# mit-acl/faster

Measured on AMD Instinct MI355X. Metric: trajectory solves/sec (whole+safe pairs) at N=10, deg=3, higher is better.
Workload: dtype f64; 1 GPU; C4: 32768 whole+safe paired solves per GPU per step (N=10 segments, deg=3, <=6 polytopes whole / <=3 safe), synthetic corridors (faster_amd/corridor.py seed 3), hand-off keeps R >= 0.05 m inside its safe corridor; pairs_per_gpu=32768, pipeline=fused, pipelines_in_flight=14, parallelism=single GPU

## Files before the change

### faster_amd/csrc/fh_solve.hip.hpp

```cpp
#pragma once
#include <hip/hip_runtime.h>
#include <stdint.h>

#include "../../include/fasterhip.h"
#include "fh_basis.hip.hpp"
#include "fh_share.hip.hpp"
#include "fh_sample.hip.hpp"

namespace fh {

#ifndef FH_LOOK_EVERY
#define FH_LOOK_EVERY 8
#endif
#ifndef FH_LOOK_EVERY_BUSY
#define FH_LOOK_EVERY_BUSY 16
#endif

#define FH_SYNC() __builtin_amdgcn_fence(__ATOMIC_SEQ_CST, "wavefront")
__device__ __forceinline__ unsigned long long pinned_clock() {
  unsigned long long t;
  asm volatile("s_memtime %0\n\ts_waitcnt lgkmcnt(0)" : "=s"(t) : : "memory");
  return t;
}
#ifdef FH_PROFILE
// ... 212 lines not shown
  const float a0 = (float)x0a, v0 = (float)x0v;
  const double c3 = (double)jerk / 6.0, c2 = (double)a0 / 2.0, c1 = (double)v0, c0 = -dx;
  double ic3 = __builtin_amdgcn_rcp(c3);
  ic3 = fma(fma(-c3, ic3, 1.0), ic3, ic3);
  const double B = c2 * ic3, C = c1 * ic3, D = c0 * ic3, B3 = B * (1.0 / 3.0);
  const double p = C - B * B3;
  const double q = 2.0 * B3 * B3 * B3 - B3 * C + D;
  const double q2 = 0.5 * q, p3 = p * (1.0 / 3.0);
  const double p27 = p3 * p3 * p3;
  const double disc = q2 * q2 + p27;
  const double scale = q2 * q2 + fabs(p27);
  const float acc = (float)(copysign(1.0, dx) * pr.a_max);
  const double qc2 = 0.5 * (double)acc;
  const double qdisc = c1 * c1 - 4.0 * qc2 * c0;
  const bool triple = !(disc > 0) && p == 0;
  const bool ill = !(fabs(disc) >= 1e-6 * scale) || (scale > 0.0 && scale < 1e-40) || !(scale < 1e280) || !(qdisc >= 0.0) || (triple && B != 0.0) ||
                   !(fabs(dx) >= 1e-30);
  if (wave_any(ill && lane < 12)) return dt_initial_exact_lanes(pr, x0, opaque(lane));
  double rj = 0.0;
  if (disc > 0) {
    const double sq = __builtin_amdgcn_sqrt(disc);
    const double u = cbrt_start(sq - q2), v = cbrt_start(-q2 - sq);
    rj = u + v - B3;
  } else if (triple) {
    rj = 0.0;
  } else {
    const double m = 2.0 * __builtin_amdgcn_sqrt(-p3);
    const float arg = fminf(1.0f, fmaxf(-1.0f, (float)(3.0 * q * __builtin_amdgcn_rcp(p * m))));
    const float rev = acos_start(arg) * (1.0f / (3.0f * 6.28318531f)) - (float)j * (1.0f / 3.0f);
    rj = m * (double)__builtin_amdgcn_cosf(rev) - B3;
  }
  if (!triple) {
#pragma unroll
    for (int it = 0; it < 3; it++) {
      const double f = ((c3 * rj + c2) * rj + c1) * rj + c0;
      const double df = (3 * c3 * rj + 2 * c2) * rj + c1;
      double r = __builtin_amdgcn_rcp(df);
      r = fma(fma(-df, r, 1.0), r, r);
      const double tn = rj - f * r;
      rj = (df == 0 || !isfinite(df) || !isfinite(tn)) ? rj : tn;
    }
  }
  if (((disc > 0 || triple) && j != 0) || j == 3) rj = 0.0;
  double ra = 0.0;
  {
    const double sr = sqrt(qdisc);
    const double qq = -0.5 * (c1 + (c1 >= 0 ? sr : -sr));
    if (qq != 0) ra = j == 0 ? qq / qc2 : (j == 1 ? c0 / qq : 0.0);
  }
  double mj = rj > 0 ? rj : INFINITY, ma = ra > 0 ? ra : INFINITY;
  mj = vmin_f64(mj, dpp_f64<0xB1, 0xf>(INFINITY, mj));
  ma = vmin_f64(ma, dpp_f64<0xB1, 0xf>(INFINITY, ma));
  mj = vmin_f64(mj, dpp_f64<0x4E, 0xf>(INFINITY, mj));
  ma = vmin_f64(ma, dpp_f64<0x4E, 0xf>(INFINITY, ma));
  const float tj = (float)(mj < INFINITY ? mj : 0.0), ta = (float)(ma < INFINITY ? ma : 0.0);
  const float ml = fmaxf(tv, fmaxf(ta, tj));
  const int mli = __float_as_int(ml);
  const float mx = fmaxf(fmaxf(0.f, __int_as_float(__builtin_amdgcn_readlane(mli, 0))),
                         fmaxf(__int_as_float(__builtin_amdgcn_readlane(mli, 4)), __int_as_float(__builtin_amdgcn_readlane(mli, 8))));
  double dt0 = (double)(mx / (float)pr.n_seg);
  if (dt0 > 10000) dt0 = 0;
  return dt0;
#endif
}

typedef const __attribute__((address_space(3))) double lds_cdouble;
__device__ __attribute__((noinline)) void write_safe_problem(const fh_problem* whole, const fh_face* wfaces, fh_problem* ps, fh_face* sfaces, lds_cdouble* x0P,
                                                             int x0_stride, int start, int cnt, double shrink, double r_margin, int lane) {
  lds_cdouble* x0V = x0P + x0_stride;
  lds_cdouble* x0A = x0V + x0_stride;
  const double x0[9] = {x0P[0], x0P[1], x0P[2], x0V[0], x0V[1], x0V[2], x0A[0], x0A[1], x0A[2]};
  const int fb = __builtin_amdgcn_readfirstlane(whole->face_begin);
  glue_write_safe<true>(wfaces, fb, whole->face_off, start, cnt, x0, shrink, r_margin, *ps, sfaces, lane, nullptr);
}

template <int NSEG>
struct Solver {
  static constexpr int NX = 3 * NSEG;
  static constexpr int NXP = (NX + 7) & ~7;
  static constexpr int KMAX = NSEG - 2;
  static constexpr int NV = 3 * KMAX;
  static constexpr int NVP = (NV + 7) & ~7;
  static constexpr int S = NVP + 1;
  static constexpr int NT = NSEG + 1;
  static constexpr int ZS = NSEG | 1;
  static_assert(NSEG >= 3, "reduced space needs N - 2 > 0 columns");
  static constexpr bool HALF = 3 * NSEG <= 32;
  static __device__ __forceinline__ double lo_sum(double v) {
    if constexpr (HALF) return half_sum(v);
    else return wave_sum(v);
  }
  static __device__ __forceinline__ double lo_min(double v) {
    if constexpr (HALF) return half_min(v);
    else return wave_min(v);
  }
  static __device__ __forceinline__ void lo_sum2(double a, double b, double& sa, double& sb) {
    if constexpr (HALF) half_sum2(a, b, sa, sb);
    else { sa = wave_sum(a); sb = wave_sum(b); }
  }
  static constexpr int RPSZ = NVP * (NVP + 1) / 2;
  static __device__ __forceinline__ int rp(int r_, int c_) { return (c_ * (c_ + 1)) / 2 + r_; }

  double *Q, *R;
  double *x, *z, *g, *d, *r, *u, *rinv;
  double *tcache, *tbnd;
  static constexpr int TC = NSEG <= 6 ? 2 : 0;
  double* xs;
  double* Zm;
  double *Pc, *Vc, *Ac;
  double* viol;
  double* xfl;
  float* tolf;
  fh_face* faces;
  int *act, *assign, *bestassign, *fullassign, *stk_seg, *stk_next, *stk_cnt, *stk_q, *stk_mask, *stk_keep, *face_off;
  int* tb;
  enum { TB_B = 0, TB_PHASE = 1, TB_F = 2, TB_TRIALS = 4, TB_BASE = 5, TB_H = 7, TB_REC = 9, TB_DEPTH0 = 10, TB_KEY = 11, TB_QE = 13,
         TB_T0 = 14, TB_WORK = 16, TB_ZN = 17, TB_NEXT = 18, TB_NEXT_EI = 20, TB_NEXT_WT = 22, TB_DONE_N = 24, TB_DONE_IT = 25, TB_SAFE = 26, TB_POOL2 = 27, TB_FRESH = 29, TB_WORDS = 30 };
  signed char* stk_order;

  static __host__ __device__ constexpr size_t lds_bytes(int max_faces) {
    return sizeof(double) * (NVP * S + RPSZ + 3 * NVP + NVP / 2 + 2 * NVP + NXP + NSEG * ZS + 3 * NT * 3 + 12 + TC * (2 * NVP + NVP / 2 + FH_MAX_POLY)) +
           sizeof(int) * (9 * NSEG + FH_MAX_POLY + 1 + TB_WORDS) + ((NSEG * FH_MAX_POLY + 15) & ~15) +
           (sizeof(fh_face) + sizeof(float)) * max_faces + 16;
  }

  double p0r, v0r, a0r;
  double xpr;
  double xj;
  double wbj, wbv, wba, wcp;
  double* bestx_g;
  double cp_r[3];
  int scan_f0, scan_F;
  int lane, N, n, q, P;
  int nx;
  int K, zc0;
  int qe;
  bool eq_ok;
  double c0;
  double box_ub;
  double gx2;
  int maxF;
  int scan_trip;
  unsigned poly_ok;
#ifdef FH_PROFILE
  unsigned long long prof[24];
  unsigned int cnt[24];
  unsigned long long take_cycles; unsigned int take_calls;
  unsigned long long glue_parts[4];
  unsigned long long pre_cycles, glue_cycles, drain_cycles;
  unsigned long long prof2[12];
  unsigned long long pre_parts[3];
#endif
  unsigned allowed_first, allowed_last;
  double h, tol, dep2;
  double vmax, amax, jmax;
  int force_final;


  __device__ void carve(unsigned char* base, int max_faces) {
    double* p = reinterpret_cast<double*>(base);
    Q = p; p += NVP * S;
    R = p; p += RPSZ;
    x = p; p += NVP;  u = p; p += NVP;
    act = reinterpret_cast<int*>(p); p += NVP / 2;
    rinv = p; p += NVP;
    g = p; p += NVP;  d = p; p += NVP;  r = d;
    xs = p; p += NXP;
    z = xs;
    static_assert(NXP >= NVP, "z aliases xs");
    Zm = p; p += NSEG * ZS;
    Pc = p; p += NT * 3;  Vc = p; p += NT * 3;  Ac = p; p += NT * 3;
    viol = g;
    static_assert(NSEG * FH_MAX_POLY <= 2 * NVP + NXP && 9 <= NVP, "scratch must fit in g,d,xs");
    xfl = p; p += 12;
    tcache = p; p += TC * SNAP_TAIL;
    tbnd = p; p += TC * FH_MAX_POLY;
    int* ip = reinterpret_cast<int*>(p);
    assign = ip; ip += NSEG;  bestassign = ip; ip += NSEG;  fullassign = ip; ip += NSEG;
    stk_seg = ip; ip += NSEG;  stk_next = ip; ip += NSEG;  stk_cnt = ip; ip += NSEG;  stk_q = ip; ip += NSEG;  stk_mask = ip; ip += NSEG;  stk_keep = ip; ip += NSEG;
    face_off = ip; ip += FH_MAX_POLY + 1;
    tb = ip; ip += TB_WORDS;
    stk_order = reinterpret_cast<signed char*>(ip);
    const size_t off = (size_t)(reinterpret_cast<unsigned char*>(ip) - base) + NSEG * FH_MAX_POLY;
    faces = reinterpret_cast<fh_face*>(base + ((off + 15) & ~(size_t)15));
    tolf = reinterpret_cast<float*>(faces + max_faces);
  }

  static constexpr int SNAP_TAIL = 2 * NVP + NVP / 2;
  static constexpr int SNAP_QOFF = (SNAP_TAIL + 127) & ~127;
  static constexpr int SNAP_BOUNDS = SNAP_TAIL, SNAP_TAIL_COPY = SNAP_TAIL + FH_MAX_POLY;
  static_assert(SNAP_TAIL + FH_MAX_POLY <= ((SNAP_TAIL + 127) & ~127), "the child bounds live in the padding behind the tail");
  static constexpr int SNAP_ROFF = SNAP_QOFF + ((NVP * S + 127) & ~127) + 128;
  static constexpr int SNAP_PADDED = SNAP_ROFF + ((RPSZ + 127) & ~127) + 128;
  __device__ __forceinline__ void copy_out(double* __restrict__ dst, const double* src, int count) const {
    const int n2 = (count + 1) >> 1;
    const double2* s2 = reinterpret_cast<const double2*>(src);
    double2* d2 = reinterpret_cast<double2*>(dst);
    for (int i = lane; i < n2; i += 64) d2[i] = s2[i];
  }
  __device__ __forceinline__ void copy_in(double* dst, const double* __restrict__ src, int count) const {
    const int n2 = (count + 1) >> 1;
    double2* d2 = reinterpret_cast<double2*>(dst);
    const double2* s2 = reinterpret_cast<const double2*>(src);
    for (int i0 = 0; i0 < n2; i0 += 256) {
      double2 t[4];
#pragma unroll
      for (int j = 0; j < 4; j++) {
        const int i = i0 + j * 64 + lane;
        t[j] = s2[i < n2 ? i : 0];
      }
#pragma unroll
      for (int j = 0; j < 4; j++) {
        const int i = i0 + j * 64 + lane;
        if (i < n2) d2[i] = t[j];
      }
    }
  }
  __device__ void snapshot_save(double* __restrict__ ws_level, int level) {
    const int lane = opaque(this->lane);
    FH_SYNC();
    if (level < TC) {
      double* tc = tcache + level * SNAP_TAIL;
      for (int i = lane; i < SNAP_TAIL; i += 64) tc[i] = x[i];
    } else {
      copy_out(ws_level, x, SNAP_TAIL);
    }
    copy_out(ws_level + SNAP_QOFF, Q, q * S);
    copy_out(ws_level + SNAP_ROFF, R, (q * (q + 1)) / 2);
    if (lane == 0) stk_keep[level] = q;
  }
  __device__ void snapshot_restore(const double* __restrict__ ws_level, int q_saved, int level) {
    const int lane = opaque(this->lane);
    const int keep0 = uniform_i32(stk_keep[level]);
    const bool intact = keep0 >= q_saved;
    const bool cached = level < TC;
    int keep = keep0 < 0 ? 0 : (keep0 > q_saved ? q_saved : keep0);
    keep &= ~1;
    if (!cached || !intact) __builtin_amdgcn_fence(__ATOMIC_SEQ_CST, "workgroup");
    if (lane < NVP)
      for (int c = q_saved; c < q; c++) Q[c * S + lane] = 0.0;
    FH_SYNC();
    constexpr int TAIL2 = SNAP_TAIL / 2, TAIL_TRIPS = (TAIL2 + 63) / 64;
    static_assert(SNAP_TAIL % 2 == 0, "the tail is copied 16 B at a time");
    if (!intact) {
      const int r0 = ((keep * (keep + 1)) / 2) & ~1;
      const int nr = (q_saved * (q_saved + 1)) / 2 - r0, nr2 = (nr + 1) >> 1;
      const double2* st2 = reinterpret_cast<const double2*>(ws_level);
      const double2* sr2 = reinterpret_cast<const double2*>(ws_level + SNAP_ROFF + r0);
      double2 tail[TAIL_TRIPS];
      if (!cached) {
#pragma unroll
        for (int j = 0; j < TAIL_TRIPS; j++) tail[j] = st2[(j * 64 + lane) < TAIL2 ? j * 64 + lane : 0];
      }
      double2 rr[2];
#pragma unroll
      for (int j = 0; j < 2; j++) rr[j] = sr2[(j * 64 + lane) < nr2 ? j * 64 + lane : 0];
      copy_in(Q + keep * S, ws_level + SNAP_QOFF + keep * S, (q_saved - keep) * S);
      if (!cached) {
#pragma unroll
        for (int j = 0; j < TAIL_TRIPS; j++)
          if (j * 64 + lane < TAIL2) reinterpret_cast<double2*>(x)[j * 64 + lane] = tail[j];
      }
#pragma unroll
      for (int j = 0; j < 2; j++)
        if (j * 64 + lane < nr2) reinterpret_cast<double2*>(R + r0)[j * 64 + lane] = rr[j];
      if (nr2 > 128) copy_in(R + r0 + 256, ws_level + SNAP_ROFF + r0 + 256, nr - 256);
    } else if (!cached) {
      copy_in(x, ws_level, SNAP_TAIL);
    }
    if (cached) {
      const double* tc = tcache + level * SNAP_TAIL;
      for (int i = lane; i < SNAP_TAIL; i += 64) x[i] = tc[i];
    }
    q = q_saved;
    if (lane == 0) stk_keep[level] = q_saved;
    FH_SYNC();
    if (lane < q_saved) rinv[lane] = 1.0 / R[rp(lane, lane)];
    FH_SYNC();
  }

  __device__ void init_problem() {
    const int lane = opaque(this->lane);
    for (int i = lane; i < NVP * S; i += 64) Q[i] = 0.0;
    for (int i = lane; i < RPSZ; i += 64) R[i] = 0.0;
    if (lane < NVP) { x[lane] = 0; g[lane] = 0; d[lane] = 0; u[lane] = 0; rinv[lane] = 0; act[lane] = 0; }
    if (lane < NXP) xs[lane] = 0;
    q = 0;
    FH_SYNC();
  }

  __device__ __forceinline__ void moments(double& dp, double& dv, double& da) const {
#pragma clang fp contract(off)
    const int lane = opaque(this->lane);
    double s0 = 0, s1 = 0, s2 = 0;
    if constexpr (HALF) {
      static_assert(!HALF || NSEG % 2 == 0, "the two halves take NSEG / 2 segments each");
      constexpr int H = NSEG / 2;
      const int row = lane & 31, hh = lane >> 5;
      const int t1 = row / 3, i = row - 3 * t1;
      const double* xh = xs + 3 * H * hh + (row < 3 * NSEG ? i : 0);
      double xr[H];
#pragma unroll
      for (int s = 0; s < H; s++) xr[s] = xh[3 * s];
      in_flight(xr);
      const int lim = opaque(t1 + 1 - H * hh);
      const double dm0 = (double)(lim - 1);
// ... 594 lines not shown
    q--;
    FH_SYNC();
  }

  __device__ void reset_qp() {
    const int lane = opaque(this->lane);
    if (lane < NVP) {
      for (int c = 0; c < q; c++) Q[c * S + lane] = 0.0;
      x[lane] = 0;
    }
    q = 0;
    FH_SYNC();
  }

  __device__ int qp_run(double ub, bool tie, int max_iters, int& iters, double& cost) {
    int it = 0;
    if (lane == 0) tb[TB_FRESH] = 0;
    bind_assignment();
    const int q0 = q;
    const int st = qp_loop(ub, tie, max_iters, it, cost);
    iters += it;
    const int qa = (q0 + q) >> 1;
    flops += (unsigned long long)(unsigned)(it + 1) * (unsigned)(2 * nx * K + 3 * (N + 1) * (5 * N + 9) + 48 * N + 18 * N + 7 * rows4 + 4 * nx + 2 * n * N) +
             (unsigned long long)(unsigned)it * (unsigned)(4 * n * qa + qa * qa + 4 * n + 5 * qa);
    return st;
  }
  __device__ int qp_loop(double ub, bool tie, int max_iters, int& it, double& cost) {
    for (;;) {
      { FH_T0(); compute_states(); FH_T1(2); }
      int id;
      double vp;
      {
        FH_T0();
        {
          const double xl = (lane < n) ? x[lane] : 0.0;
          double x2, l1x;
          lo_sum2(xl * xl, fabs(xj), x2, l1x);
          cost = c0 + x2;
          if (!(cost <= box_ub) || cost > l1x * (jmax + tol) * (1.0 + 1e-9)) {
            const int al = lane < NVP ? act[lane] : 0;
            conflict = wave_or((lane < q && (al >> 24) == K_POLY) ? (1u << ((al >> 16) & 31)) : 0u);
            return 1;
          }
          if (cost > ub || (tie && cost == ub)) return 2;
        }
        bool cbad;
        scan(id, vp, cbad);
        FH_T1(3);
        if (cbad) return 1;
        if (id < 0) return 0;
      }
      double gg;
      { FH_T0(); gg = build_g(id); FH_T1(4); }
      double up = 0;
      for (;;) {
        if (++it > max_iters) return 3;
        double dc, zi, zz, rc;
        { FH_T0(); zz = project(gg, dc, zi); FH_T1(5); }
        FH_T0();
        rc = backsolve(dc);
        const bool dependent = zz <= dep2 * gx2;
        double ratio = INFINITY;
        if (lane < q && rc > 0) ratio = u[lane] / rc;
        const double t1 = wave_any(ratio < INFINITY) ? lo_min(ratio) : INFINITY;
        const int kb = (t1 < INFINITY) ? first_lane(ratio == t1) : -1;
        if (kb < 0 && dependent) {
          const int al = lane < NVP ? act[lane] : 0;
          bool in = lane < q && rc != 0.0;
          if (vp * (1.0 - 1e-9) > tol) {
            double cn = 0.0;
            const int cl = lane < q ? lane : 0;
            for (int r_ = 0; r_ < q; r_++) {
              const double v = R[rp(min(r_, cl), cl)];
              cn += (r_ <= cl) ? v * v : 0.0;
            }
            const double xl = (lane < n) ? x[lane] : 0.0;
            const double xn = sqrt(wave_sum(xl * xl));
            const double thr = 1e-9 * vp / ((double)q * (xn + sqrt((double)nx) * jmax));
            in = in && fabs(rc) * sqrt(cn) > thr;
          }
          conflict = wave_or((in && (al >> 24) == K_POLY) ? (1u << ((al >> 16) & 31)) : 0u) |
                     ((id >> 24) == K_POLY ? (1u << ((id >> 16) & 31)) : 0u);
          return 1;
        }
        const double t2 = dependent ? INFINITY : vp / zz;
        const double t = fmin(t1, t2);
        if (lane < q) u[lane] -= t * rc;
        up += t;
        if (!dependent) {
          if (lane < n) x[lane] -= t * zi;
          vp -= t * zz;
        }
        FH_T1(6);
        if (t2 <= t1) {
          FH_T0();
          add_row(id, zi, zz, dc, up);
#ifdef FH_QMAX_STAT
          qmax = max(qmax, q);
#endif
          FH_T1(7);
          break;
        }
        FH_SYNC();
        { FH_T0(); drop_row(kb); FH_T1(8); }
      }
    }
  }

  __device__ __forceinline__ unsigned allowed_mask(int t) const {
    unsigned m = P ? (((1u << P) - 1u) & poly_ok) : 0u;
    if (t == 0) m &= allowed_first;
    if (t == N - 1) m &= allowed_last;
    return m;
  }

  template <class PR>
  __device__ void screen_constant_rows(const PR& pr) {
    const int lane = opaque(this->lane);
    allowed_first = allowed_last = 0xffffffffu;
    if (P == 0) return;
    double c0[9], cN[9];
    {
      const double h3 = h / 3.0, h23 = 2.0 * h / 3.0, h26 = h * h / 6.0;
#pragma unroll
      for (int i = 0; i < 3; i++) {
        const double p0 = Pc[i], v0 = Vc[i], a0 = Ac[i];
        const double pf = xfl[i], vf = xfl[3 + i], af = xfl[6 + i];
        c0[i] = p0; c0[3 + i] = p0 + v0 * h3; c0[6 + i] = p0 + v0 * h23 + a0 * h26;
        cN[i] = pf; cN[3 + i] = pf - vf * h3; cN[6 + i] = pf - vf * h23 + af * h26;
      }
    }
    const int nf = face_off[P];
    unsigned bad = 0u;
    for (int fb = 0; fb < nf; fb += 64) {
      const int f = fb + lane;
      const bool valid = f < nf;
      const fh_face fc = faces[valid ? f : 0];
      double w0 = -INFINITY, wN = -INFINITY;
#pragma unroll
      for (int k = 0; k < 3; k++) {
        w0 = vmax_f64(w0, fma(fc.a[0], c0[3 * k], fma(fc.a[1], c0[3 * k + 1], fma(fc.a[2], c0[3 * k + 2], fc.b))));
        wN = vmax_f64(wN, fma(fc.a[0], cN[3 * k], fma(fc.a[1], cN[3 * k + 1], fma(fc.a[2], cN[3 * k + 2], fc.b))));
      }
      int pf = 0;
      for (int j = 1; j < P; j++) pf += (f >= face_off[j]) ? 1 : 0;
      if (valid) bad |= ((w0 > 0.0) ? (1u << pf) : 0u) | ((wN > 0.0) ? (256u << pf) : 0u);
    }
    bad = wave_or(bad);
    allowed_first = ~(bad & 255u);
    if (force_final) allowed_last = ~((bad >> 8) & 255u);
  }

  template <class PR>
  __device__ int analyze(const PR& pr, bool root) {
    const int lane = opaque(this->lane);
    if (P == 0) {
      if (lane < N) fullassign[lane] = -1;
      FH_SYNC();
      return -1;
    }
    const int sh = HALF ? (N * P <= 16 ? 2 : (N * P <= 32 ? 1 : 0)) : 0;
    const int trip = (maxF + (1 << sh) - 1) >> sh;
    for (int pair0 = 0; pair0 < N * P; pair0 += 64 >> sh) {
      const int pair = pair0 + (lane >> sh);
      const int r0 = (lane & ((1 << sh) - 1)) * trip;
      const bool live = pair < N * P;
      const int t = live ? pair / P : 0, p = live ? pair - t * P : 0;
      const bool need = live && assign[t] < 0 && ((allowed_mask(t) >> p) & 1u);
      const int fp0 = face_off[p], Fp = need ? face_off[p + 1] - fp0 : 0;
      const bool mine = r0 == 0 || r0 < Fp;
      const int f0 = fp0 + (mine ? r0 : 0), F = mine ? Fp - r0 : 0;
      double c[12];
      {
        double st[12];
#pragma unroll
        for (int i = 0; i < 3; i++) { st[i] = Pc[3 * t + i]; st[3 + i] = Vc[3 * t + i]; st[6 + i] = Ac[3 * t + i]; st[9 + i] = Pc[3 * t + 3 + i]; }
        in_flight(st);
#pragma unroll
        for (int k = 0; k < 4; k++)
#pragma unroll
          for (int i = 0; i < 3; i++) c[3 * k + i] = cp_of(k, st[i], st[3 + i], st[6 + i], st[9 + i]);
      }
      const int fl = F > 0 ? F - 1 : 0;
      const fh_face* fp = faces + f0;
      double worst = -INFINITY;
      for (int fb = 0; fb < trip; fb += 4) {
        fh_face fc[4];
#pragma unroll
        for (int j = 0; j < 4; j++) fc[j] = fp[min(fb + j, fl)];
#pragma unroll
        for (int j = 0; j < 4; j++) {
#pragma unroll
          for (int k = 0; k < 4; k++)
            worst = vmax_f64(worst, fma(fc[j].a[0], c[3 * k], fma(fc[j].a[1], c[3 * k + 1], fma(fc[j].a[2], c[3 * k + 2], fc[j].b))));
        }
      }
      if (!need || !mine) worst = -INFINITY;
      if constexpr (HALF) worst = slices_max(sh, worst);
      if (live && r0 == 0) viol[t * FH_MAX_POLY + p] = (assign[t] < 0 && !need) ? INFINITY : worst;
    }
    FH_SYNC();
    double score = -INFINITY;
    if (lane < N) {
      int full = assign[lane];
      if (full < 0) {
        double mn = INFINITY;
        for (int p = 0; p < P; p++) {
          const double v = viol[lane * FH_MAX_POLY + p];
          if (v < mn) { mn = v; full = p; }
        }
        score = mn;
      }
      fullassign[lane] = full;
    }
    const double bw = wave_max_nonneg(score);
    FH_SYNC();
    if (!(bw > 0.0)) return -1;
    if (root) {
      const bool ends_outside = __ballot(lane == N - 1 && score > 0.0) != 0ull;
      const bool far_outside = __ballot(lane == N - 1 && score > 1.2 * (vmax * vmax) / (2.0 * amax)) != 0ull;
      if (lane == 0) tb[TB_QE] = ends_outside ? (1 << 16) : 0;
      return first_lane(far_outside ? score > 0.0 : score == bw);
    }
    const bool earliest = (uniform_i32(tb[TB_QE]) >> 16) != 0;
    return first_lane(earliest ? score > 0.0 : score == bw);
  }

  int rec;
  int depth0;
  unsigned long long cur_key;
  unsigned long long best_key;
  unsigned long long flops;
  int rows4;
  int fin_solved;
  double fin_dt;
  unsigned conflict;
  unsigned allinf;

  __device__ __forceinline__ void tb_put64(int at, unsigned long long v) { tb[at] = (int)(unsigned)v; tb[at + 1] = (int)(unsigned)(v >> 32); }
  __device__ __forceinline__ unsigned long long tb_get64(int at) const {
    return ((unsigned long long)(unsigned)uniform_i32(tb[at + 1]) << 32) | (unsigned)uniform_i32(tb[at]);
  }

  static __device__ __forceinline__ unsigned long long uniform_u64(unsigned long long v) {
    const unsigned lo = (unsigned)__builtin_amdgcn_readfirstlane((int)(unsigned)v);
    const unsigned hi = (unsigned)__builtin_amdgcn_readfirstlane((int)(unsigned)(v >> 32));
    return ((unsigned long long)hi << 32) | lo;
  }
  static __device__ __forceinline__ unsigned long long f64_bits(double v) { return (unsigned long long)__double_as_longlong(v); }
  static __device__ __forceinline__ double bits_f64(unsigned long long v) { return __longlong_as_double((long long)v); }

  __device__ __forceinline__ void copy_out_shared(double* dst, const double* __restrict__ src, int count_) const {
    const int count = (count_ + 1) & ~1;
    for (int i0 = 0; i0 < count; i0 += 256) {
      double t[4];
#pragma unroll
      for (int j = 0; j < 4; j++) {
        const int i = i0 + j * 64 + lane;
        t[j] = src[i < count ? i : 0];
      }
#pragma unroll
      for (int j = 0; j < 4; j++) {
        const int i = i0 + j * 64 + lane;
        if (i < count) wt_store(dst + i, t[j]);
      }
    }
  }
  __device__ __forceinline__ void copy_in_shared(double* __restrict__ dst, const double* src, int count_) const {
    const int count = (count_ + 1) & ~1;
    for (int i0 = 0; i0 < count; i0 += 256) {
      double t[4];
#pragma unroll
      for (int j = 0; j < 4; j++) {
        const int i = i0 + j * 64 + lane;
        t[j] = cc_load(src + (i < count ? i : 0));
      }
#pragma unroll
      for (int j = 0; j < 4; j++) {
        const int i = i0 + j * 64 + lane;
        if (i < count) dst[i] = t[j];
      }
    }
  }
  __device__ __forceinline__ void pack_bytes(int v, int count, unsigned long long& lo, unsigned long long& hi) const {
    const unsigned byte = (lane < 16) ? ((unsigned)((lane < count ? v : -1) & 0xff) << (8 * (lane & 3))) : 0u;
    unsigned w[4];
#pragma unroll
    for (int k = 0; k < 4; k++) w[k] = wave_or((lane >> 2) == k ? byte : 0u);
    lo = ((unsigned long long)w[1] << 32) | w[0];
    hi = ((unsigned long long)w[3] << 32) | w[2];
  }
  static __device__ __forceinline__ int unpack_byte(unsigned long long lo, unsigned long long hi, int t) {
    return (int)(signed char)(unsigned char)((t < 8 ? lo : hi) >> (8 * (t & 7)));
  }

  __device__ int look_around(const ShareArgs& sa, int local_nodes, int iters_so_far = 0) {
    FH_SP_T0();
    int flags = 0;
    if (lane == 0) {
      const unsigned long long t_start = ((unsigned long long)(unsigned)tb[TB_T0 + 1] << 32) | (unsigned)tb[TB_T0];
      const unsigned long long ei = ald(reinterpret_cast<unsigned long long*>(&sa.ctl->error));
      const unsigned long long wt = ald(reinterpret_cast<unsigned long long*>(&sa.ctl->wait_ticket));
      const unsigned int waiters = (unsigned int)wt, tail = (unsigned int)(wt >> 32);
      unsigned int stop = (unsigned int)ei | (unsigned int)(ei >> 32);
      if (!stop) {
        if (sa.deadline_ticks && wall_ticks() - t_start > sa.deadline_ticks) stop = 2u;
// ... 469 lines not shown
      Ti[5] = qmax;
#endif
      T[3] = solved ? factor : 0.0;
      T[4] = dt;
      T[5] = solved ? cost : 0.0;
      tb[TB_WORK] += iters;
    }
    fin_solved = solved ? 1 : 0;
    fin_dt = dt;
    fin_rows = rows;
    FH_SYNC();
  }
  __device__ __forceinline__ void flush_result(fh_result& res) {
    const int lane = opaque(this->lane);
    const int rows = fin_rows;
    const int body = (RES_HEAD + 12 * rows) >> 1;
    unsigned char* out = reinterpret_cast<unsigned char*>(&res);
    const double2* T2 = reinterpret_cast<const double2*>(Q);
    for (int c = lane; c <= body; c += 64) {
#ifdef FH_SHARE_PROFILE
      if (c == (RES_HEAD + (FH_MAX_SEG - 1) * 12 + 8) / 2) continue;
#endif
      const double2 v = T2[c];
      *reinterpret_cast<double2*>(out + (c < body ? (size_t)16 * c : offsetof(fh_result, assign))) = v;
    }
  }
  int fin_rows;
#ifdef FH_QMAX_STAT
  int qmax;
#endif

  template <class PW, class PS>
  __device__ __forceinline__ int handoff_onchip(const PW& pw, const PS& ps, const fh_face* __restrict__ wfaces, double feas_tol, double r_frac, double shrink,
                                                int max_safe_poly, double r_margin, const fh_pair_rule& rule, const UnknownGrid* ug,
                                                unsigned long long* probe) {
    const int lane = opaque(this->lane);
    forget_lane_state();
    ProblemView pv;
    pv.n_seg = N; pv.n_poly = P; pv.face_begin = pw.face_begin; pv.dc = pw.dc; pv.a_max = pw.a_max;
    pv.x0[0] = uniform_f64(Pc[0]); pv.x0[1] = uniform_f64(Pc[1]); pv.x0[2] = uniform_f64(Pc[2]);
    pv.face_off = face_off;
    ResultView rv;
    rv.solved = fin_solved; rv.dt = fin_dt;
    rv.coeff = reinterpret_cast<const double (*)[12]>(Q + RES_HEAD);
    typedef const __attribute__((address_space(4))) double cdouble;
    const double xfv = (reinterpret_cast<cdouble*>(&ps.xf[0]))[lane < 9 ? lane : 0];
    fh_state R;
    {
      const bool found = glue_find_r(pv, rv, r_frac, rule, lane, ug, R, probe);
      if (lane == 0) tb[TB_SAFE] = found ? 0 : 0x200;
    }
    if (lane < 9) {
      const double rv9[9] = {R.pos[0], R.pos[1], R.pos[2], R.vel[0], R.vel[1], R.vel[2], R.accel[0], R.accel[1], R.accel[2]};
      double v = rv9[0];
#pragma unroll
      for (int j = 1; j < 9; j++) v = lane == j ? rv9[j] : v;
      *x0_slot(lane) = v;
      xfl[lane] = xfv;
    }
    const double Rp[3] = {R.pos[0], R.pos[1], R.pos[2]};
    const bool keep_r = r_margin >= 0.0;
    const double test_shrink = keep_r ? 0.0 : shrink;
    const double slack_ok = keep_r ? 1e-7 : 0.0;
    const int Pw = P, fb = pv.face_begin;
    const int nf = Pw ? uniform_i32(face_off[Pw]) : 0;
    double worst = -INFINITY;
    fh_face fc0 = {{0.0, 0.0, 0.0}, 0.0};
    for (int f0 = 0; f0 < nf; f0 += 64) {
      const int f = f0 + lane;
      double v = -INFINITY;
      int pf = -1;
      if (f < nf) {
        const fh_face fc = wfaces[fb + f];
        if (f0 == 0) fc0 = fc;
        v = glue_face_test(fc, glue_face_norm(fc), Rp, test_shrink);
        pf = 0;
        for (int p = 1; p < Pw; p++) pf += (f >= face_off[p]) ? 1 : 0;
      }
      for (int p = 0; p < Pw; p++) {
        const double m = wave_max(pf == p ? v : -INFINITY);
        worst = lane == p ? fmax(worst, m) : worst;
      }
    }
    if (probe) probe[2] = __builtin_readcyclecounter();
    int start = first_lane(lane < Pw && worst <= slack_ok);
    if (start < 0) {
      const double least = wave_min(lane < Pw ? worst : INFINITY);
      start = first_lane(lane < Pw && worst == least);
      if (start < 0) start = 0;
    }
    int cnt = Pw - start;
    if (cnt > max_safe_poly) cnt = max_safe_poly;
    if (Pw == 0) cnt = 0;
    const int src0 = cnt ? uniform_i32(face_off[start]) : 0;
    const int total = cnt ? uniform_i32(face_off[start + cnt]) - src0 : 0;
    const int noff = (cnt && lane <= FH_MAX_POLY) ? face_off[start + (lane < cnt ? lane : cnt)] - src0 : 0;
    const int first_end = __builtin_amdgcn_readlane(noff, 1);
    FH_SYNC();
    unsigned badpoly = 0u;
    for (int f0 = 0; f0 < src0 + total; f0 += 64) {
      const int f = f0 + lane, j = f - src0;
      const bool on = j >= 0 && j < total;
      bool degenerate_violated = false;
      fh_face fc = fc0;
      if (f0 > 0 && on) fc = wfaces[fb + f];
      if (on) {
        fc.b = glue_face_b(fc, glue_face_norm(fc), Rp, shrink, keep_r, j < first_end, r_margin);
        stage_face(fc, feas_tol, j, degenerate_violated);
      }
      if (wave_any(degenerate_violated)) {
        int pf = 0;
        for (int p = 1; p < cnt; p++) pf += (j >= __builtin_amdgcn_readlane(noff, p)) ? 1 : 0;
        for (int p = 0; p < cnt; p++)
          if (wave_any(degenerate_violated && pf == p)) badpoly |= 1u << p;
      }
    }
    if (probe) probe[3] = __builtin_readcyclecounter();
    if (lane <= FH_MAX_POLY) face_off[lane] = noff;
    {
      int mf = 0;
      for (int p = 0; p < cnt; p++) mf = max(mf, __builtin_amdgcn_readlane(noff, p + 1) - __builtin_amdgcn_readlane(noff, p));
      maxF = mf;
    }
    P = cnt;
    poly_ok = ~badpoly;
    if (lane == 0) tb[TB_SAFE] |= start;
    FH_SYNC();
    return (uniform_i32(tb[TB_SAFE]) & 0x200) ? 2 : 1;
  }

  template <class PR>
  __device__ __forceinline__ bool x0_outside_box(const PR& pr) const {
    bool x0bad = false;
    for (int i = 0; i < 3; i++) x0bad |= (fabs(uniform_f64(Vc[i])) - vmax > tol) || (fabs(uniform_f64(Ac[i])) - amax > tol);
    return x0bad;
  }

  template <class PR>
  __device__ int search(const PR& pr, const fh_params& par, const ShareArgs& sa, double* __restrict__ ws, int entry,
                        double& best_cost, int& nodes, int& iters) {
    int depth = 0;
    int status_limit = 0;
    bool backtrack = false;
    bool carry_inf = false;
    unsigned carry = 0u;
    allinf = 0u;
    if (entry == 0) {
      FH_U0();
      best_cost = INFINITY;
      best_key = ~0ull;
      cur_key = 0ull;
      depth0 = 0;
      if (lane < NSEG) assign[lane] = -1;
      if (x0_outside_box(pr)) return FH_ST_INFEASIBLE;
      {
        FH_T0();
        screen_constant_rows(pr);
        FH_T1(13);
      }
      if (P > 0) {
        if (allowed_mask(0) == 0u || allowed_mask(N - 1) == 0u) return FH_ST_INFEASIBLE;
        const unsigned long long pins = (unsigned long long)pr.pin[0] | ((unsigned long long)pr.pin[1] << 32);
        bool pin_bad = false;
        for (int t = 0; t < N; t++) {
          const int v = (int)((pins >> (4 * t)) & 15ull);
          if (v && !((allowed_mask(t) >> (v - 1)) & 1u)) pin_bad = true;
        }
        if (pin_bad) return FH_ST_INFEASIBLE;
        FH_SYNC();
        if (lane < N) {
          const int v = (int)((pins >> (4 * lane)) & 15ull);
          if (v) assign[lane] = v - 1;
          else if (lane == 0 || lane == N - 1) {
            const unsigned m = allowed_mask(lane);
            if ((m & (m - 1u)) == 0u) assign[lane] = __builtin_ctz(m);
          }
        }
        FH_SYNC();
      }
      reset_qp();
      qe = 0;
      if (lane == 0) tb[TB_QE] = 0;
      FH_U1(0);
      if (!eq_ok) return FH_ST_INFEASIBLE;
    } else {
      depth = 1;
      backtrack = true;
    }
    int local_nodes = 0;
    for (;;) {
      if (backtrack) {
        FH_U0();
        bool have_node = false;
        while (depth > 0) {
          const int d_ = depth - 1;
          const int seg = stk_seg[d_];
          if (carry_inf) {
            if (!((carry >> seg) & 1u)) {
              FH_SYNC();
              if (lane == 0) assign[seg] = -1;
              depth--;
              FH_SYNC();
              continue;
            }
            if (lane == 0) stk_mask[d_] |= (int)carry;
          } else {
            allinf &= ~(1u << d_);
          }
          carry_inf = false;
          const int nx = stk_next[d_];
          if (nx < stk_cnt[d_]) {
            if (sa.child_bound && best_cost < INFINITY) {
              double lb;
              if (d_ < TC) {
                FH_SYNC();
                lb = uniform_f64(tbnd[d_ * FH_MAX_POLY + uniform_i32(nx)]);
              } else {
                __builtin_amdgcn_fence(__ATOMIC_SEQ_CST, "workgroup");
                lb = uniform_f64(ws[(size_t)d_ * SNAP_PADDED + SNAP_BOUNDS + uniform_i32(nx)]);
              }
              const int shp = 3 * (15 - (depth0 + d_));
              const unsigned long long ckey = ((cur_key >> (shp + 3)) << (shp + 3)) | ((unsigned long long)(unsigned)uniform_i32(nx) << shp);
              const double ubp = best_cost * (1.0 - par.mip_gap);
              if (lb > ubp || (ckey > best_key && lb == ubp)) {
                FH_SYNC();
                if (lane == 0) stk_next[d_] = nx + 1;
                FH_SYNC();
                continue;
              }
            }
            FH_SYNC();
            if (lane == 0) { stk_next[d_] = nx + 1; assign[seg] = stk_order[d_ * FH_MAX_POLY + nx]; }
            { FH_T0(); snapshot_restore(ws + (size_t)d_ * SNAP_PADDED, stk_q[d_], d_); FH_T1(11); }
            const int sh = 3 * (15 - (depth0 + d_));
            cur_key = ((cur_key >> (sh + 3)) << (sh + 3)) | ((unsigned long long)nx << sh);
            have_node = true;
            break;
          }
          FH_SYNC();
          if ((allinf >> d_) & 1u) {
            carry_inf = true;
            carry = (unsigned)uniform_i32(stk_mask[d_]) & ~(1u << seg);
          }
          if (lane == 0) assign[seg] = -1;
          depth--;
          FH_SYNC();
        }
        FH_U1(1);
        if (!have_node) break;
      }
      backtrack = true;
#ifdef FH_PROFILE
      const unsigned long long u2__ = __builtin_readcyclecounter();
#endif
      if (local_nodes >= par.max_nodes) { status_limit = FH_ST_NODE_LIMIT; break; }
      if (par.max_work > 0 && iters >= par.max_work) { status_limit = FH_ST_ITER_LIMIT; break; }
      local_nodes++;
      if ((local_nodes & (rec >= 0 ? (sa.look_mask >> 1) : sa.look_mask)) == 0 || (rec >= 0 && local_nodes == 1 && (entry == 1 || trial + 1 < trial_end))) {
        FH_T0();
        int fl = look_around(sa, local_nodes, iters);
        if (fl & 1) { status_limit = FH_ST_INTERRUPTED; break; }
        if (sa.enabled) give_tickets(sa);
        if ((fl & 2) && ((fl & 4) ? (rec >= 0 || nodes + local_nodes >= sa.min_nodes) : (nodes + local_nodes >= sa.giant_nodes || (fl & 8)))) {
          for (int pass = 0; pass < 2; pass++) {
            if (pass == 1) {
              const int fl2 = look_around(sa, 1);
              if (!(fl2 & 2)) break;
              if (trial + 1 < trial_end) {
                donate_trials(sa, pr, best_cost, (fl2 >> 8) & 63);
                break;
              }
              if (rec < 0) break;
            }
            if (depth > 0) donate(sa, ws, depth, best_cost);
          }
        }
        FH_T1(16);
      }
      if (rec >= 0) {
        const unsigned long long r = uniform_u64(ald(&(sa.recs + rec)->inc_rank));
        const int rt = rank_trial(r);
        if (rt < trial) break;
        if (rt == trial) {
          const double gc = rank_cost_up(r);
          if (gc < best_cost) { best_cost = gc; best_key = ~0ull; }
        }
      }
      double cost = 0;
#ifdef FH_PROFILE
      const unsigned long long u3__ = __builtin_readcyclecounter();
      prof2[2] += u3__ - u2__;
#endif
      const int st = qp_run(best_cost * (1.0 - par.mip_gap), cur_key > best_key, par.max_iters, iters, cost);
#ifdef FH_PROFILE
      prof2[3] += __builtin_readcyclecounter() - u3__;
#endif
      if (st == 3) { status_limit = FH_ST_ITER_LIMIT; break; }
      carry_inf = st == 1;
      carry = conflict;
      if (st == 0) {
        int bseg;
        { FH_T0(); bseg = analyze(pr, entry == 0 && local_nodes == 1); FH_T1(9); }
        if (bseg < 0) {
          FH_T0();
          if (cost < best_cost || (cost == best_cost && cur_key < best_key)) {
            best_cost = cost;
            best_key = cur_key;
            if (lane < n) bestx_g[lane] = x[lane];
            if (lane < N) bestassign[lane] = fullassign[lane];
            if (lane == 0) tb[TB_FRESH] = 1;
            FH_SYNC();
            if (rec >= 0) publish_incumbent(sa, cost);
          }
          FH_T1(21);
// ... 145 lines not shown
  return sa.compact_results ? NSEG : FH_MAX_SEG;
#endif
}

template <int NSEG, class SV, class PR>
__device__ __forceinline__ bool run_problem(SV& sv, const PR& pr, const fh_face* __restrict__ gfaces, int max_faces,
                            const fh_params& par, const ShareArgs& sa, const double* __restrict__ basis, double* __restrict__ ws, int entry,
                            bool interrupted, int staged, bool defer_store, fh_result& res) {
  const int lane = sv.lane;
  sv.fin_solved = 0;
  const int rows = result_rows<NSEG>(sa);
#ifdef FH_SHARE_PROFILE
  const unsigned long long sp_tp__ = wall_ticks();
#endif
#ifdef FH_PROFILE
  const unsigned long long tstart__ = pinned_clock();
  for (int i = 0; i < 24; i++) { sv.prof[i] = 0; sv.cnt[i] = 0; }
  for (int i = 0; i < 8; i++) sv.prof2[i] = 0;
  sv.prof2[8] = sv.pre_parts[0]; sv.prof2[9] = sv.pre_parts[1]; sv.prof2[10] = sv.pre_parts[2];
  sv.pre_parts[0] = sv.pre_parts[1] = sv.pre_parts[2] = 0;
  sv.prof[18] = sv.glue_cycles; sv.cnt[18] = sv.glue_cycles ? 1 : 0; sv.glue_cycles = 0;
  sv.prof[19] = sv.pre_cycles; sv.cnt[19] = sv.pre_cycles ? 1 : 0; sv.pre_cycles = 0;
  sv.prof[23] = sv.drain_cycles; sv.cnt[23] = sv.drain_cycles ? 1 : 0; sv.drain_cycles = 0;
  sv.prof[22] = sv.take_cycles; sv.cnt[22] = sv.take_calls; sv.take_cycles = 0; sv.take_calls = 0;
  const unsigned long long gp0__ = sv.glue_parts[0], gp1__ = sv.glue_parts[1], gp2__ = sv.glue_parts[2], gp3__ = sv.glue_parts[3];
  sv.glue_parts[0] = sv.glue_parts[1] = sv.glue_parts[2] = sv.glue_parts[3] = 0;
#endif
  sv.forget_lane_state();
#ifdef FH_QMAX_STAT
  sv.qmax = 0;
#endif
  FH_SYNC();
  double x0xf = 0.0;
  if (staged == 0) {
    typedef const __attribute__((address_space(4))) double cdouble;
    static_assert(offsetof(fh_problem, xf) == offsetof(fh_problem, x0) + 9 * sizeof(double), "x0 and xf are adjacent");
    x0xf = (reinterpret_cast<cdouble*>(&pr.x0[0]))[lane < 18 ? lane : 0];
  }
  bool bad = interrupted;
  if (entry == 0 && !bad) bad = bad_scalars(pr, NSEG, staged ? sv.P : (int)pr.n_poly) || (staged == 0 && bad_corridor(pr, max_faces));
  fh_face fc_first = {{0.0, 0.0, 0.0}, 0.0};
  if (staged == 0 && !bad) {
    const int nf_ = pr.n_poly ? pr.face_off[pr.n_poly] : 0;
    if (lane < nf_) fc_first = gfaces[pr.face_begin + lane];
  }
  if (staged == 0) {
    if (lane < 9) *sv.x0_slot(lane) = x0xf;
    else if (lane < 18) sv.xfl[lane - 9] = x0xf;
    FH_SYNC();
  }
  if (entry == 0 && !bad) {
    const double v = lane < 9 ? *sv.x0_slot(lane) : sv.xfl[lane < 18 ? lane - 9 : 0];
    bad = wave_any(!isfinite(v));
  }
  if (entry == 0 && bad) {
    sv.N = 0; sv.flops = 0ull; sv.P = 0; sv.maxF = 0;
    if (lane <= FH_MAX_POLY) sv.face_off[lane] = 0;
    sv.emit_result(false, 0, interrupted ? FH_ST_INTERRUPTED : FH_ST_BAD_INPUT, 0, 0, 0.0, 0.0, 0.0, rows);
    if (!defer_store) sv.flush_result(res);
    return true;
  }

#ifdef FH_SHARE_PROFILE
  if (entry == 0 && lane == 0) {
    const unsigned long long t00 = ((unsigned long long)(unsigned)sv.tb[sv.TB_T0 + 1] << 32) | (unsigned)sv.tb[sv.TB_T0];
    res.coeff[FH_MAX_SEG - 1][8] = (double)(wall_ticks() - t00) / 100.0;
  }
#endif
  sv.N = pr.n_seg;
  sv.nx = 3 * pr.n_seg;
  sv.zc0 = pr.force_final_pos ? 3 : 2;
  sv.K = max(pr.n_seg - sv.zc0, 0);
  sv.n = 3 * sv.K;
  if (staged == 0) sv.P = pr.n_poly;
  sv.tol = par.feas_tol;
  sv.dep2 = par.dep_tol * par.dep_tol;
  sv.vmax = pr.v_max; sv.amax = pr.a_max; sv.jmax = pr.j_max;
  sv.box_ub = (double)(3 * pr.n_seg) * pr.j_max * pr.j_max * (1.0 + 1e-9);
  sv.force_final = pr.force_final_pos;
  sv.init_problem();
#ifdef FH_PROFILE
  sv.prof2[4] = pinned_clock() - tstart__;
#endif
  const double* bt = reinterpret_cast<const double*>(sv.uniform_u64((unsigned long long)(basis + (size_t)(pr.n_seg - 1) * BT_STRIDE)));
  if (uniform_i32(sv.tb[sv.TB_ZN]) != pr.n_seg) {
    const int nn = pr.n_seg * pr.n_seg;
    for (int idx = lane; idx < nn; idx += 64) {
      const int s_ = idx / pr.n_seg;
      sv.Zm[s_ * sv.ZS + (idx - s_ * pr.n_seg)] = bt[BT_Z + idx];
    }
    if (lane == 0) sv.tb[sv.TB_ZN] = pr.n_seg;
  }
#ifdef FH_PROFILE
  sv.prof2[5] = pinned_clock() - tstart__ - sv.prof2[4];
#endif

  if (staged == 0) {
    const int nf = pr.n_poly ? pr.face_off[pr.n_poly] : 0;
    if (lane <= FH_MAX_POLY) sv.face_off[lane] = pr.face_off[lane];
    {
      int mf = 0;
      for (int p = 0; p < pr.n_poly; p++) mf = max(mf, pr.face_off[p + 1] - pr.face_off[p]);
      sv.maxF = mf;
    }
    unsigned badpoly = 0u;
    for (int f0_ = 0; f0_ < nf; f0_ += 64) {
      const int f = f0_ + lane;
      bool degenerate_violated = false;
      if (f < nf) sv.stage_face(f0_ == 0 ? fc_first : gfaces[pr.face_begin + f], par.feas_tol, f, degenerate_violated);
      if (wave_any(degenerate_violated)) {
        int pf = 0;
        for (int p = 0; p < pr.n_poly; p++) pf = (f >= pr.face_off[p]) ? p : pf;
        for (int p = 0; p < pr.n_poly; p++)
          if (wave_any(degenerate_violated && pf == p)) badpoly |= 1u << p;
      }
    }
    sv.poly_ok = ~badpoly;
  }
  FH_SYNC();

#ifdef FH_PROFILE
  sv.prof[0] = pinned_clock() - tstart__;
#endif
  const X0Lds x0l = {sv.Pc, 3 * sv.NT};
  const double dt0 = dt_initial(pr, x0l, lane);
  const double base = fmax(dt0, 2 * pr.dc);
#ifdef FH_PROFILE
  sv.prof[14] = pinned_clock() - tstart__ - sv.prof[0]; sv.cnt[14] = 1;
#endif
  int trials = entry ? uniform_i32(sv.tb[sv.TB_TRIALS]) - 1 : 0, nodes = 0, iters = 0, status = FH_ST_INFEASIBLE;
  bool solved = false;
  double f = entry ? sv.bits_f64(sv.tb_get64(sv.TB_F)) : pr.f_init, dt = 0, factor = 0, cost = 0;
  sv.rec = entry ? uniform_i32(sv.tb[sv.TB_REC]) : -1;
  sv.trial_end = entry == 0 ? 0x7fffffff : (entry == 2 ? uniform_i32(sv.tb[sv.TB_DEPTH0]) : 0);
  sv.flops = 0ull;
  if (lane == 0) sv.tb_put64(sv.TB_BASE, sv.f64_bits(base));
  unsigned limit = 0u;
  bool last_trial = false;
#ifdef FH_PROFILE
  const unsigned long long tloop__ = pinned_clock();
#endif
  for (;;) {
    if (entry != 1) {
      if (!(f <= pr.f_final) || trials >= sv.trial_end) break;
      if (sv.rec >= 0 && rank_trial(sv.uniform_u64(ald(&(sa.recs + sv.rec)->inc_rank))) <= trials) break;
      dt = f * base;
    } else {
      dt = sv.bits_f64(sv.tb_get64(sv.TB_H));
    }
    sv.trial = trials;
    trials++;
    last_trial = !(f + pr.f_inc <= pr.f_final);
    sv.h = dt;
    if (lane == 0) sv.tb_put64(sv.TB_F, sv.f64_bits(f));
    bool early_inf;
    { FH_T0(); early_inf = sv.setup_trial(pr, bt, entry != 1);
#ifdef FH_PROFILE
      sv.prof[1] += __builtin_readcyclecounter() - t0__; sv.cnt[1] += 1;
#endif
    }
    double best = INFINITY;
    if (entry == 1) sv.install_frame(pr, sa, best);
#ifdef FH_SHARE_PROFILE
    const bool sp_taken__ = entry != 0;
    const unsigned long long sp_ts__ = wall_ticks();
    const int sp_n0__ = nodes;
    if (sp_taken__ && lane == 0) { aadd(&sa.ctl->prof2[0], sp_ts__ - sp_tp__); aadd(&sa.ctl->prof2[1], 1ull); }
#endif
#ifdef FH_PROFILE
    const unsigned long long ts0__ = __builtin_readcyclecounter();
#endif
    int st;
    if (early_inf && !sv.x0_outside_box(pr) && par.max_nodes > 0 && !(par.max_work > 0 && iters >= par.max_work)) {
      st = FH_ST_INFEASIBLE;
      nodes += 1;
      if ((trials & 7) == 0) {
        unsigned int stop = 0u;
        if (lane == 0) {
          const unsigned long long ei = ald(reinterpret_cast<unsigned long long*>(&sa.ctl->error));
          stop = (unsigned int)ei | (unsigned int)(ei >> 32);
          if (!stop && sa.deadline_ticks) {
            const unsigned long long t_start = ((unsigned long long)(unsigned)sv.tb[sv.TB_T0 + 1] << 32) | (unsigned)sv.tb[sv.TB_T0];
            if (wall_ticks() - t_start > sa.deadline_ticks) { stop = 2u; ast(&sa.ctl->interrupted, 2u); }
          }
        }
        if (uniform_i32((int)stop) != 0) st = FH_ST_INTERRUPTED;
      }
    } else
      st = sv.search(pr, par, sa, ws, entry == 1 ? 1 : 0, best, nodes, iters);
#ifdef FH_PROFILE
    sv.prof[15] += __builtin_readcyclecounter() - ts0__; sv.cnt[15] += 1;
#endif
#ifdef FH_SHARE_PROFILE
    if (sp_taken__ && lane == 0) { aadd(&sa.ctl->prof2[2], wall_ticks() - sp_ts__); aadd(&sa.ctl->prof2[3], (unsigned long long)(nodes - sp_n0__)); }
#endif
    entry = 0;
    limit = (st == FH_ST_NODE_LIMIT || st == FH_ST_ITER_LIMIT || st == FH_ST_INTERRUPTED) ? (unsigned)st : 0u;
    if (sv.rec < 0) {
      status = limit ? (int)limit : (best < INFINITY ? FH_ST_OPTIMAL : FH_ST_INFEASIBLE);
      if (status == FH_ST_OPTIMAL) {
        solved = true;
        factor = f;
        cost = best;
        break;
      }
      if (status == FH_ST_INTERRUPTED || (par.max_work > 0 && status == FH_ST_ITER_LIMIT)) break;
      f = f + pr.f_inc;
      continue;
    }
    if (limit && limit != FH_ST_INTERRUPTED) sv.note_limited(sa, limit);
    if (trials >= sv.trial_end || limit == FH_ST_INTERRUPTED || best < INFINITY) break;
    f = f + pr.f_inc;
  }
#ifdef FH_PROFILE
  sv.prof2[6] = pinned_clock() - tloop__;
  const unsigned long long tpost__ = pinned_clock();
#endif
  if (sv.rec >= 0) {
    if (!sv.finish_part(sa, nodes, iters, limit, last_trial)) return false;
    const ShareRec* R_ = sa.recs + sv.rec;
    const unsigned long long r = sv.uniform_u64(ald(&R_->inc_rank));
    const unsigned long long limited = sv.uniform_u64(ald(&R_->limited));
    const unsigned int last_status = (unsigned int)uniform_i32((int)ald(&R_->last_status));
    const int wt = rank_trial(r);
    solved = r != FH_RANK_NONE && last_status != FH_ST_INTERRUPTED && !((limited >> (wt < 63 ? wt : 63)) & 1ull);
    if (solved) {
      status = FH_ST_OPTIMAL;
      trials = wt + 1;
      cost = uniform_f64(sv.bits_f64(ald(&R_->inc_cost)));
      factor = uniform_f64(sv.bits_f64(ald(reinterpret_cast<const unsigned long long*>(&R_->inc_f))));
      dt = uniform_f64(sv.bits_f64(ald(reinterpret_cast<const unsigned long long*>(&R_->inc_h))));
      const unsigned long long alo = sv.uniform_u64(ald(&R_->assign_lo)), ahi = sv.uniform_u64(ald(&R_->assign_hi));
      if (lane < sv.n) sv.bestx_g[lane] = cc_load(&R_->x[lane]);
      if (lane < NSEG) sv.bestassign[lane] = sv.unpack_byte(alo, ahi, lane);
      sv.h = dt;
      (void)sv.setup_trial(pr, bt);
    } else {
      const unsigned int limit_kind = (unsigned int)uniform_i32((int)ald(&R_->limit_kind));
      status = (r != FH_RANK_NONE && last_status != FH_ST_INTERRUPTED) ? (int)(limit_kind ? limit_kind : (unsigned)FH_ST_NODE_LIMIT)
                                                                       : (last_status ? (int)last_status : FH_ST_INFEASIBLE);
      trials = 0;
      for (double fk = pr.f_init; fk <= pr.f_final; fk = fk + pr.f_inc) {
        trials++;
        dt = fk * base;
      }
    }
  }

#ifdef FH_PROFILE
  const unsigned long long tres__ = pinned_clock();
  sv.prof2[7] = tres__ - tpost__;
#endif
  if (solved) {
    FH_SYNC();
    __builtin_amdgcn_fence(__ATOMIC_SEQ_CST, "workgroup");
    if (lane < sv.NVP) sv.x[lane] = (lane < sv.n) ? sv.bestx_g[lane] : 0.0;
    FH_SYNC();
    sv.compute_states();
    FH_SYNC();
    if (lane < sv.NXP) sv.xs[lane] = (lane < sv.nx) ? sv.xj : 0.0;
    FH_SYNC();
  }
  sv.emit_result(solved, trials, status, nodes, iters, factor, dt, cost, rows);
#ifdef FH_PROFILE
  sv.prof[17] = pinned_clock() - tres__; sv.cnt[17] = 1;
  sv.prof[12] = pinned_clock() - tstart__;
  if (lane < 12 && sv.N <= FH_MAX_SEG - 4) {
    unsigned long long pv = 0, pw = 0;
    unsigned int cv = 0, cw = 0;
    for (int i = 0; i < 12; i++) { pv = (i == lane) ? sv.prof[i] : pv; cv = (i == lane) ? sv.cnt[i] : cv; }
    for (int i = 0; i < 12; i++) { pw = (i == lane) ? sv.prof[12 + i] : pw; cw = (i == lane) ? sv.cnt[12 + i] : cw; }
    double* Tc = sv.Q + sv.RES_HEAD;
    Tc[(FH_MAX_SEG - 1) * 12 + lane] = (double)pv;
    Tc[(FH_MAX_SEG - 2) * 12 + lane] = (double)cv;
    Tc[(FH_MAX_SEG - 3) * 12 + lane] = (double)pw;
    Tc[(FH_MAX_SEG - 4) * 12 + lane] = (double)cw;
    if (lane < 4) Tc[(FH_MAX_SEG - 5) * 12 + lane] = (double)(lane == 0 ? gp0__ : (lane == 1 ? gp1__ : (lane == 2 ? gp2__ : gp3__)));
    if (sv.N <= FH_MAX_SEG - 6) {
      unsigned long long pu = 0;
      for (int i = 0; i < 12; i++) pu = (i == lane) ? sv.prof2[i] : pu;
      Tc[(FH_MAX_SEG - 6) * 12 + lane] = (double)pu;
    }
  }
  FH_SYNC();
#endif
  if (!defer_store) sv.flush_result(res);
#ifdef FH_SHARE_PROFILE
  if (lane == 0 && sv.N < FH_MAX_SEG) {
    const unsigned long long t00 = ((unsigned long long)(unsigned)sv.tb[sv.TB_T0 + 1] << 32) | (unsigned)sv.tb[sv.TB_T0];
    res.coeff[FH_MAX_SEG - 1][11] = (double)(wall_ticks() - t00) / 100.0;
    res.coeff[FH_MAX_SEG - 1][10] = (double)(sp_tp__ - t00) / 100.0;
    res.coeff[FH_MAX_SEG - 1][9] = sv.rec >= 0 ? 1.0 : 0.0;
  }
#endif
  return true;
}

struct SolveArgs {
  int n, max_faces;
  fh_params par;
  double* workspace;
  const double* basis;
  ShareArgs sa;
  fh_problem* safe;
  fh_face* sfaces;
  fh_result* sres;
  double r_frac, shrink, r_margin;
  int max_safe_poly, pad;
  fh_pair_rule rule;
  UnknownGrid unknown;
  const int* order;
};

template <int NSEG, bool PAIRS, int WPS = FH_WAVES_PER_SIMD, bool UNK = false>
__global__ void __launch_bounds__(64, WPS) solve_kernel(const fh_problem* __restrict__ problems, const fh_face* __restrict__ faces,
                                                   fh_result* __restrict__ results, SolveArgs ka) {
  extern __shared__ __attribute__((aligned(16))) unsigned char smem[];
  typedef Solver<NSEG> SolverT;
  SolverT sv;
  sv.carve(smem, ka.max_faces);
  sv.lane = threadIdx.x;
  sv.q = 0;
  sv.qe = 0;
  if (threadIdx.x == 0) { sv.tb[sv.TB_ZN] = 0; sv.tb_put64(sv.TB_NEXT, 0ull); sv.tb_put64(sv.TB_POOL2, 0ull); sv.tb_put64(sv.TB_NEXT_EI, 0ull); sv.tb_put64(sv.TB_NEXT_WT, 0ull); sv.tb[sv.TB_DONE_N] = 0; sv.tb[sv.TB_DONE_IT] = 0; }
  const ShareArgs& sa = ka.sa;
  double* ws = ka.workspace + (size_t)blockIdx.x * ((size_t)NSEG * (size_t)Solver<NSEG>::SNAP_PADDED + 64);
  sv.bestx_g = ws + (size_t)NSEG * (size_t)Solver<NSEG>::SNAP_PADDED;
  if (threadIdx.x == 0) {
    sv.tb_put64(sv.TB_T0, wall_ticks());
    aadd(&sa.ctl->started, 1u);
  }
  bool tickets_left = true;
#ifdef FH_SHARE_PROFILE
  unsigned long long sp_dry__ = 0;
#endif
#ifdef FH_PROFILE
  sv.pre_cycles = 0; sv.glue_cycles = 0; sv.drain_cycles = 0; sv.take_cycles = 0; sv.take_calls = 0;
  sv.glue_parts[0] = sv.glue_parts[1] = sv.glue_parts[2] = sv.glue_parts[3] = 0;
  sv.pre_parts[0] = sv.pre_parts[1] = sv.pre_parts[2] = 0;
  for (int i = 0; i < 12; i++) sv.prof2[i] = 0;
#endif
  for (;;) {
    int entry = 0, unit = 0, phase = 0;
    bool interrupted = false;
    sv.forget_lane_state();
#ifdef FH_PROFILE
    const unsigned long long tpre__ = pinned_clock();
#endif
    int pool_next = uniform_i32(sv.tb[sv.TB_NEXT]), pool_end = uniform_i32(sv.tb[sv.TB_NEXT + 1]);
    bool frame_pending = true, fresh_words = false;
    if (pool_next >= pool_end && pool_end > 0) {
      const int p2a = uniform_i32(sv.tb[sv.TB_POOL2]), p2b = uniform_i32(sv.tb[sv.TB_POOL2 + 1]);
      if (p2a < p2b) {
        pool_next = p2a; pool_end = p2b;
        FH_SYNC();
        if (threadIdx.x == 0) { sv.tb[sv.TB_NEXT] = p2a; sv.tb[sv.TB_NEXT + 1] = p2b; sv.tb_put64(sv.TB_POOL2, 0ull); }
        FH_SYNC();
      }
    }
    if (tickets_left && pool_next < pool_end) {
// ... 298 lines not shown
```

Baseline: 20.82 million pairs/s.

## Certify infeasibility of all later time-scale trials and skip them early

Adds a per-face certificate check: when the first or last segment has no allowed polytope, it tests whether the endpoint state stays outside each face for any larger time step, using the Bezier control-point bounds. If every candidate polytope is certified violated, the remaining time-factor trials are skipped, with only the trial counter and dt advanced. This removes repeated setup and search over trials that cannot succeed. The cost is an extra face scan on the infeasible path. Correctness depends on the monotonicity argument holding, and the tolerance margin could wrongly prune a feasible trial.

```diff
diff --git a/faster_amd/csrc/fh_solve.hip.hpp b/faster_amd/csrc/fh_solve.hip.hpp
--- a/faster_amd/csrc/fh_solve.hip.hpp
+++ b/faster_amd/csrc/fh_solve.hip.hpp
@@ -388,6 +388,7 @@
   unsigned long long pre_parts[3];
 #endif
   unsigned allowed_first, allowed_last;
+  bool no_later_trial;
   double h, tol, dep2;
   double vmax, amax, jmax;
   int force_final;
@@ -1288,6 +1289,45 @@
   }
 
   template <class PR>
+  __device__ void no_later_trials(const PR& pr) {
+    const int lane = opaque(this->lane);
+    const double hF = pr.f_final * bits_f64(tb_get64(TB_BASE));
+    const double h3 = h / 3.0, h23 = 2.0 * h / 3.0, h26 = h * h / 6.0;
+    double e0[9], eN[9], mag0 = 1.0, magN = 1.0;
+#pragma unroll
+    for (int i = 0; i < 3; i++) {
+      e0[i] = Pc[i]; e0[3 + i] = Vc[i]; e0[6 + i] = Ac[i];
+      eN[i] = xfl[i]; eN[3 + i] = -xfl[3 + i]; eN[6 + i] = xfl[6 + i];
+      mag0 += fabs(e0[i]) + hF * (fabs(e0[3 + i]) + hF * fabs(e0[6 + i]));
+      magN += fabs(eN[i]) + hF * (fabs(eN[3 + i]) + hF * fabs(eN[6 + i]));
+    }
+    const int nf = face_off[P];
+    unsigned cert = 0u;
+    for (int fb = 0; fb < nf; fb += 64) {
+      const int f = fb + lane;
+      const bool valid = f < nf;
+      const fh_face fc = faces[valid ? f : 0];
+      bool c[2];
+#pragma unroll
+      for (int e = 0; e < 2; e++) {
+        const double* xe = e ? eN : e0;
+        const double m = 1e-9 * ((e ? magN : mag0) + fabs(fc.b));
+        const double val0 = fma(fc.a[0], xe[0], fma(fc.a[1], xe[1], fma(fc.a[2], xe[2], fc.b)));
+        const double s = fma(fc.a[0], xe[3], fma(fc.a[1], xe[4], fc.a[2] * xe[5]));
+        const double w = fma(fc.a[0], xe[6], fma(fc.a[1], xe[7], fc.a[2] * xe[8]));
+        const double val1 = val0 + h3 * s, val2 = val0 + h23 * s + h26 * w;
+        c[e] = val0 > m || (val1 > m && s >= 0.0) || (val2 > m && w >= 0.0 && (2.0 / 3.0) * s + h3 * w >= 0.0);
+      }
+      int pf = 0;
+      for (int j = 1; j < P; j++) pf += (f >= face_off[j]) ? 1 : 0;
+      if (valid) cert |= (c[0] ? (1u << pf) : 0u) | (c[1] ? (256u << pf) : 0u);
+    }
+    cert = wave_or(cert);
+    const unsigned cand = ((1u << P) - 1u) & poly_ok;
+    no_later_trial = (cand & ~cert) == 0u || (force_final && (cand & ~(cert >> 8)) == 0u);
+  }
+
+  template <class PR>
   __device__ int analyze(const PR& pr, bool root) {
     const int lane = opaque(this->lane);
     if (P == 0) {
@@ -2063,14 +2103,20 @@
       cur_key = 0ull;
       depth0 = 0;
       if (lane < NSEG) assign[lane] = -1;
-      if (x0_outside_box(pr)) return FH_ST_INFEASIBLE;
+      if (x0_outside_box(pr)) {
+        no_later_trial = true;
+        return FH_ST_INFEASIBLE;
+      }
       {
         FH_T0();
         screen_constant_rows(pr);
         FH_T1(13);
       }
       if (P > 0) {
-        if (allowed_mask(0) == 0u || allowed_mask(N - 1) == 0u) return FH_ST_INFEASIBLE;
+        if (allowed_mask(0) == 0u || allowed_mask(N - 1) == 0u) {
+          no_later_trials(pr);
+          return FH_ST_INFEASIBLE;
+        }
         const unsigned long long pins = (unsigned long long)pr.pin[0] | ((unsigned long long)pr.pin[1] << 32);
         bool pin_bad = false;
         for (int t = 0; t < N; t++) {
@@ -2522,6 +2568,7 @@
     trials++;
     last_trial = !(f + pr.f_inc <= pr.f_final);
     sv.h = dt;
+    sv.no_later_trial = false;
     if (lane == 0) sv.tb_put64(sv.TB_F, sv.f64_bits(f));
     bool early_inf;
     { FH_T0(); early_inf = sv.setup_trial(pr, bt, entry != 1);
@@ -2576,6 +2623,13 @@
       }
       if (status == FH_ST_INTERRUPTED || (par.max_work > 0 && status == FH_ST_ITER_LIMIT)) break;
       f = f + pr.f_inc;
+      if (sv.trial_end == 0x7fffffff && status == FH_ST_INFEASIBLE && sv.no_later_trial) {
+        for (; f <= pr.f_final; f = f + pr.f_inc) {
+          trials++;
+          dt = f * base;
+        }
+        break;
+      }
       continue;
     }
     if (limit && limit != FH_ST_INTERRUPTED) sv.note_limited(sa, limit);
```

New measurement: 20.92 million pairs/s (median of 6 runs). No clear change (+0.5%).
